# JiLiBIT/LIO-SLAM

Measured on AMD Instinct MI355X. Metric: scan-to-map registrations/sec, 64x1800 scan vs 200-keyframe map; pose RMSE, higher is better.
Workload: dtype f32

## Files before the change

include/liogpu.h:

```cpp
#ifndef LIOGPU_H
#define LIOGPU_H

#include <stddef.h>
#include <stdint.h>

#ifdef __cplusplus
extern "C" {
#endif

#define LIO_VERSION 102
#define LIO_MAX_ITERS 32

enum {
    LIO_OK               = 0,
    LIO_TOO_FEW_POINTS   = 1,
    LIO_TOO_FEW_CORR     = 2,
    LIO_ERR_ARG          = -1,
    LIO_ERR_HIP          = -2,
    LIO_ERR_CAPACITY     = -3,
    LIO_ERR_NO_MAP       = -4,
    LIO_ERR_NO_DEVICE    = -5
};

typedef struct lio_s2m_config {
// ... 56 lines not shown
    float   launch_ms[LIO_MAX_ITERS];
    int32_t launch_active[LIO_MAX_ITERS];
    int64_t point_iters;
    int64_t n_map;
    int64_t n_cells;
    int32_t pipeline;
    int32_t multi_iterations;
    int32_t multi_stream_syncs;
    int32_t multi_event_waits;
    int32_t multi_exchange;
    int32_t persist_fallbacks;
    int32_t map_x_sub;
    int32_t map_tight_tables;
    int32_t map_first_try;
    float   map_pts_per_cell;
} lio_s2m_profile;

typedef struct lio_s2m_handle lio_s2m_handle;

int  lio_version(void);
void lio_s2m_default_config(lio_s2m_config *cfg);
const char *lio_last_error(void);

int  lio_s2m_create(const lio_s2m_config *cfg, lio_s2m_handle **out);
void lio_s2m_destroy(lio_s2m_handle *h);

int  lio_s2m_set_map(lio_s2m_handle *h, const void *pts, size_t n, size_t stride_bytes);

int  lio_s2m_register(lio_s2m_handle *h, const void *scan, size_t n, size_t stride_bytes,
                      float pose[6], lio_s2m_result *res);
// ... 334 lines not shown
```

lio-slam_amd/api.py:

```python
import ctypes as C
import os
import subprocess

import numpy as np

_HERE = os.path.dirname(os.path.abspath(__file__))
LIO_MAX_ITERS = 32
STATUS_NAMES = {0: "OK", 1: "TOO_FEW_POINTS", 2: "TOO_FEW_CORR", -1: "ERR_ARG", -2: "ERR_HIP",
                -3: "ERR_CAPACITY", -4: "ERR_NO_MAP", -5: "ERR_NO_DEVICE"}


class LioError(RuntimeError):
    pass


class S2MConfig(C.Structure):
    _fields_ = [
        ("k", C.c_int32), ("max_sq_dist", C.c_float),
        ("plane_tol", C.c_double), ("weight", C.c_double), ("min_s", C.c_double),
        ("min_corr", C.c_int32), ("max_iters", C.c_int32), ("eig_thresh", C.c_float),
        ("conv_deg", C.c_double), ("conv_cm", C.c_double),
        ("min_scan_pts", C.c_int32), ("jacobian_mode", C.c_int32), ("force_all_iters", C.c_int32),
        ("device_id", C.c_int32), ("cell_size", C.c_float), ("max_batch", C.c_int32),
        ("max_scan_pts", C.c_int32), ("record_corr_iter", C.c_int32), ("kernel_variant", C.c_int32),
# ... 12 lines not shown
        ("matP", C.c_float * 36), ("AtA", C.c_float * 36), ("AtB", C.c_float * 6),
        ("pose_iter", (C.c_float * 6) * LIO_MAX_ITERS),
    ]


class S2MProfile(C.Structure):
    _fields_ = [
        ("map_build_ms", C.c_float), ("map_upload_ms", C.c_float), ("n_launches", C.c_int32),
        ("n_units", C.c_int32), ("unit_iters", C.c_int32),
        ("launch_ms", C.c_float * LIO_MAX_ITERS), ("launch_active", C.c_int32 * LIO_MAX_ITERS),
        ("point_iters", C.c_int64),
        ("n_map", C.c_int64), ("n_cells", C.c_int64),
        ("pipeline", C.c_int32), ("multi_iterations", C.c_int32), ("multi_stream_syncs", C.c_int32),
        ("multi_event_waits", C.c_int32), ("multi_exchange", C.c_int32), ("persist_fallbacks", C.c_int32),
        ("map_x_sub", C.c_int32), ("map_tight_tables", C.c_int32), ("map_first_try", C.c_int32), ("map_pts_per_cell", C.c_float),
    ]


class DeskewConfig(C.Structure):
    _fields_ = [
        ("N_SCAN", C.c_int32), ("downsampleRate", C.c_int32), ("point_filter_num", C.c_int32),
        ("lidarMinFront", C.c_float), ("lidarMinBack", C.c_float),
        ("lidarMinLeft", C.c_float), ("lidarMinRight", C.c_float),
        ("lidarMaxRange", C.c_float), ("lidarMaxIntensity", C.c_float),
        ("deskew_flag", C.c_int32), ("device_id", C.c_int32),
    ]


class RangeImageConfig(C.Structure):
    _fields_ = [("N_SCAN", C.c_int32), ("Horizon_SCAN", C.c_int32), ("downsampleRate", C.c_int32),
# ... 1029 lines not shown
```

lio-slam_amd/csrc/lio_handle.h:

```cpp
#pragma once
#include <hip/hip_runtime.h>
#include <stdio.h>
#include <string.h>
#include <string>
#include <vector>

#include "../../include/liogpu.h"
#include "lio_kernels.h"
#include "lio_pool.h"
#include "lio_types.h"

int lio_pc2_check_xyz(const lio_pc2_layout* L);
void lio_raw_ws_free(struct LioRawWs* ws);

struct lio_s2m_handle {
    ~lio_s2m_handle();
    lio_s2m_config cfg;
    LioConsts c;
    hipStream_t stream = nullptr;
    bool own_stream = true;

    bool has_map = false;
    size_t n_map = 0;
    LioDevBuf<float> d_mx, d_my, d_mz;
// ... 12 lines not shown
    std::vector<LioScanState> h_state;
    std::vector<LioBlockDesc> v_blocks, v_prep;
    std::vector<LioScanTiles> v_tiles;
    std::vector<LioBlockDesc> v_blocks_sorted;
    std::vector<int> v_order, v_first, v_first_orig;
    bool defer_sync = false;
    bool async_upload = false;
    LioDevBuf<float> d_poses;
    const float* reg_pose = nullptr;
    bool pose_in_state = false;
    LioDevBuf<float> d_summary;
    LioPinned<float> h_summary;
    bool host_state_stale = false;
    LioDevBuf<LioBlockDesc> d_blocks;
    int n_blocks = 0, ppt = 1, max_blk = 1;
    LioDevBuf<double> d_partials;
    LioDevBuf<unsigned> d_arrive;
    bool poses_set = false, ran = false;
    LioDevBuf<LioScanTiles> d_tiles;
    LioDevBuf<LioBlockDesc> d_prep_blocks;
    LioDevBuf<int> d_key_of, d_key_count, d_key_start, d_key_tiles, d_tmp_idx, d_perm;
    LioDevBuf<float> d_block_box;
    bool has_block_box = false;
    LioDevBuf<unsigned char> d_blk_skip;
    LioDevBuf<int> d_big_list;
    LioDevBuf<unsigned> d_scan_bbox;
    LioPinned<unsigned> h_scan_bbox;
    bool sorted = false;
    const unsigned char* last_stage = nullptr;
    size_t last_stride = 0, last_xyz_off = 0;
// ... 6 lines not shown
    unsigned persist_spin_max = 0;
    int persist_withhold = -1;
    lio_s2m_handle* map_src = nullptr;
    unsigned long long map_epoch = 0;
    LioDevBuf<float> d_nn_cache;
    LioDevBuf<long long> d_stamps;
    LioDevBuf<unsigned> d_gen;
    LioDevBuf<double> d_spec_sums;
    unsigned gen_epoch = 0;
    int n_cu = 0;
    bool run_persist = false;
    bool soa_valid = true;
    hipGraph_t graph = nullptr;
    hipGraphExec_t graph_exec = nullptr;
    bool graph_dirty = true;
    int graph_chunk = 0, graph_blocks = 0, graph_ppt = 0;
    LioIterParams graph_params;
    int units_this_run = 0, unit_iters = 1;

    LioDevBuf<unsigned char> d_rec_flag;
    LioDevBuf<float> d_rec_coeff;
    LioDevBuf<int> d_rec_nn;

    struct LioMulti* multi = nullptr;

    bool run_pending = false, run_graph = false, run_has_c = false;
    int run_next = 0, run_units = 0, run_look = 0;
    LioIterParams run_P, run_Pc;

    LioShard shard{};
// ... 21 lines not shown
```

lio-slam_amd/csrc/lio_kernels.h:

```cpp
#pragma once
#include <hip/hip_runtime.h>
#include "lio_types.h"

struct LioIterParams {
    LioGrid grid;
    LioShard shard;
    LioConsts c;
    const float4* map_sorted;
    const float4* map_xyz4;
    const int* cell_start;
    const float4* nbr_pts;
    const int* nbr_start;
    const float* sx;
    const float* sy;
    const float* sz;
    const int* perm;
    LioScanState* state;
    const LioBlockDesc* blocks;
    double* partials;
    unsigned* arrive;
    int max_blk;
    int xcd_remap;
    int* n_active;
    double* sums_out;
// ... 6 lines not shown
};

void lio_launch_aos_to_soa(const void* src, size_t stride, int n, float* x, float* y, float* z,
                           float4* xyz4, hipStream_t s);
void lio_launch_map_bbox(const float* x, const float* y, const float* z, int n, unsigned* bbox, hipStream_t s);
void lio_launch_map_build(const LioGrid& g, const float* x, const float* y, const float* z, int n,
                          int* cell_of, int* cell_count, int* cell_start, int* tile_sums,
                          float4* sorted, int* nbr_start, float4* nbr_pts, int* nbr_slot, bool with_cell_sorted, hipStream_t s);
void lio_launch_map_cell_sort(const LioGrid& g, const float* x, const float* y, const float* z, int n, int* cell_of, int* cell_count,
                              int* cell_start, int* tile_sums, float4* sorted, hipStream_t s);
void lio_launch_map_occupancy(const LioGrid& g, const float* x, const float* y, const float* z, int n, int* flags, hipStream_t s);
int  lio_scan_tiles(int n_cells);
void lio_launch_init_state(LioScanState* st, int n_scans, float* poses, bool from_state, const LioConsts& c,
                           int* n_active, hipStream_t s);
void lio_launch_iterate(const LioIterParams& P, int n_blocks, int ppt, bool stage, hipStream_t s, bool corner = false);
void lio_launch_persist(const LioIterParams& P, int n_blocks, unsigned* gen, unsigned epoch, const unsigned char* stage, size_t stride,
                        int n_scans, unsigned* spec, double* spec_sums, const float* poses0, unsigned spin_max, int withhold_wg, hipStream_t s);
void lio_launch_pack_summary(const LioScanState* st, int n_scans, float* out, hipStream_t s);
void lio_launch_apply(LioScanState* st, int n_scans, const double* sums, size_t slot_stride, int n_slots, const LioConsts& c,
                      int* n_active, hipStream_t s);
void lio_launch_shard_cull(const LioIterParams& P, int n_ranks, int rank, int halo, const int* bounds, const float* block_box,
                           int n_blocks, unsigned char* skip, hipStream_t s);
void lio_launch_block_boxes(const LioBlockDesc* blocks, int n_blocks, const LioScanState* st, const float* sx, const float* sy,
                            const float* sz, float* box, hipStream_t s);
void lio_launch_scan_sort_lds(const void* stage, size_t stride, const LioScanState* st, int n_scans, int max_pts, float tile0,
                              int shard_axis, int* perm, float* x, float* y, float* z, hipStream_t s);
void lio_launch_scan_bbox(const void* stage, size_t stride, const LioBlockDesc* prep_blocks, int n_prep_blocks,
                          const LioScanState* st, unsigned* bbox, hipStream_t s);
void lio_launch_scan_tile_sort(const void* stage, size_t stride, int total_pts,
                               const LioBlockDesc* prep_blocks, int n_prep_blocks,
// ... 8 lines not shown
```

lio-slam_amd/csrc/lio_kernels.hip:

```cpp
#include <hip/hip_runtime.h>
#include "lio_types.h"
#include "lio_device_math.h"
#include "lio_kernels.h"

#include "lio_s2m_device.h"
#include "lio_scan2.h"
#include "lio_wg.h"

__global__ void k_aos_to_soa(const unsigned char* __restrict__ src, size_t stride, int n,
                             float* __restrict__ x, float* __restrict__ y, float* __restrict__ z,
                             float4* __restrict__ xyz4 )
{
    int i = blockIdx.x * blockDim.x + threadIdx.x;
    if (i >= n) return;
    const float* p = reinterpret_cast<const float*>(src + (size_t)i * stride);
    const float a = p[0], b = p[1], c = p[2];
    x[i] = a; y[i] = b; z[i] = c;
    if (xyz4) xyz4[i] = make_float4(a, b, c, 0.0f);
}

__global__ void k_xyzi4_to_soa(const float4* __restrict__ src, int n, float* __restrict__ x, float* __restrict__ y,
                               float* __restrict__ z, float4* __restrict__ xyz4)
{
    const int i = blockIdx.x * blockDim.x + threadIdx.x;
// ... 476 lines not shown
    const int li = bd.first + (int)threadIdx.x;
    const int base = st[bd.scan].offset;
    float mn[3] = { INFINITY, INFINITY, INFINITY }, mx[3] = { -INFINITY, -INFINITY, -INFINITY };
    if (li < st[bd.scan].n_pts) {
        const float v[3] = { sx[base + li], sy[base + li], sz[base + li] };
#pragma unroll
        for (int a = 0; a < 3; ++a) if (fabsf(v[a]) <= 3.0e38f) { mn[a] = v[a]; mx[a] = v[a]; }
    }
    __shared__ LioWgBoxLds<LIO_BLOCK / 64> s_box;
    float lo, hi;
    lio_wg_box(mn, mx, s_box, lo, hi);
    if (threadIdx.x < 3) {
        const int a = threadIdx.x;
        float* o = box + (size_t)((base + bd.first) / LIO_BLOCK + bd.scan) * 6;
        o[a] = lo; o[3 + a] = hi;
    }
}

struct LioShardPlan {
    int n_ranks;
    int rank;
    int halo;
    int bounds[9];
};

__global__ __launch_bounds__(256) void k_shard_cull(LioIterParams P, LioShardPlan plan, const float* __restrict__ block_box, int n_blocks,
                                                    unsigned char* __restrict__ skip)
{
    const int lane = threadIdx.x & 63, c = lane & 7;
    const int i = (blockIdx.x * 4 + (int)(threadIdx.x >> 6)) * 8 + (lane >> 3);
// ... 520 lines not shown
    if (stage) {
        switch (ppt) {
        case 1: hipLaunchKernelGGL((k_s2m_iterate<1, true, false>), gr, bl, 0, s, P); break;
        case 2: hipLaunchKernelGGL((k_s2m_iterate<2, true, false>), gr, bl, 0, s, P); break;
        default: hipLaunchKernelGGL((k_s2m_iterate<4, true, false>), gr, bl, 0, s, P); break;
        }
    } else {
        switch (ppt) {
        case 1: hipLaunchKernelGGL((k_s2m_iterate<1, false, false>), gr, bl, 0, s, P); break;
        case 2: hipLaunchKernelGGL((k_s2m_iterate<2, false, false>), gr, bl, 0, s, P); break;
        default: hipLaunchKernelGGL((k_s2m_iterate<4, false, false>), gr, bl, 0, s, P); break;
        }
    }
}

void lio_launch_pack_summary(const LioScanState* st, int n_scans, float* out, hipStream_t s)
{
    hipLaunchKernelGGL(k_s2m_pack_summary, dim3((n_scans + 255) / 256), dim3(256), 0, s, st, n_scans, out);
}

void lio_launch_apply(LioScanState* st, int n_scans, const double* sums, size_t slot_stride, int n_slots, const LioConsts& c,
                      int* n_active, hipStream_t s)
{
    hipLaunchKernelGGL(k_s2m_apply, dim3(n_scans), dim3(64), 0, s, st, n_scans, sums, slot_stride, n_slots, c, n_active);
}

void lio_launch_shard_cull(const LioIterParams& P, int n_ranks, int rank, int halo, const int* bounds, const float* block_box,
                           int n_blocks, unsigned char* skip, hipStream_t s)
{
    if (n_blocks <= 0) return;
// ... 63 lines not shown
```

lio-slam_amd/csrc/liogpu_api.hip:

```cpp
#include <hip/hip_runtime.h>
#include <math.h>
#include <stdio.h>
#include <string.h>
#include <algorithm>
#include <chrono>
#include <exception>
#include <memory>
#include <mutex>
#include <vector>

#include "lio_handle.h"
#include "lio_multi.h"
#include "lio_wg.h"


static thread_local char g_last_error[512];

int lio_fail(int code, const char* what, hipError_t e)
{
    if (e != hipSuccess) snprintf(g_last_error, sizeof(g_last_error), "%s: %s", what, hipGetErrorString(e));
    else snprintf(g_last_error, sizeof(g_last_error), "%s", what);
    return code;
}

// ... 71 lines not shown
}

static int lio_s2m_init_resources(lio_s2m_handle* h)
{
    HIPCHK(hipStreamCreateWithFlags(&h->stream, hipStreamNonBlocking));
    for (int i = 0; i < LIO_MAX_ITERS; ++i) {
        HIPCHK(hipEventCreate(&h->ev_beg[i]));
        HIPCHK(hipEventCreate(&h->ev_end[i]));
        HIPCHK(hipEventCreateWithFlags(&h->ev_chk[i], hipEventDisableTiming));
    }
    HIPCHK(h->h_active.grow(LIO_MAX_ITERS, LIO_MAX_ITERS));
    HIPCHK(hipEventCreate(&h->ev_map[0]));
    HIPCHK(hipEventCreate(&h->ev_map[1]));
    HIPCHK(hipEventCreate(&h->ev_mapl[0]));
    HIPCHK(hipEventCreate(&h->ev_mapl[1]));
    HIPCHK(h->d_bbox.grow(6, 1.0, 0));
    HIPCHK(h->d_active.grow(1, 1.0, 0));
    hipDeviceProp_t prop;
    if (hipGetDeviceProperties(&prop, h->cfg.device_id) == hipSuccess) h->n_cu = prop.multiProcessorCount;
    (void)hipGetLastError();
    return LIO_OK;
}

extern "C" int lio_s2m_create(const lio_s2m_config* cfg, lio_s2m_handle** out)
try {
    if (!cfg || !out) return lio_fail(LIO_ERR_ARG, "null argument");
    if (cfg->k != 5) return lio_fail(LIO_ERR_ARG, "only k = 5 is supported (MO:1631)");
    if (cfg->max_iters < 1 || cfg->max_iters > LIO_MAX_ITERS) return lio_fail(LIO_ERR_ARG, "max_iters out of range");
    if (!(cfg->max_sq_dist > 0.0f)) return lio_fail(LIO_ERR_ARG, "max_sq_dist must be positive");
    if (cfg->x_sub != 0 && cfg->x_sub != 1 && cfg->x_sub != 2 && cfg->x_sub != 4 && cfg->x_sub != 8)
// ... 30 lines not shown
    (void)hipSetDevice(h->cfg.device_id);
    (void)hipStreamSynchronize(h->stream);
    delete h;
}

lio_s2m_handle::~lio_s2m_handle()
{
    delete multi;
    lio_s2m_destroy(corner);
    lio_raw_ws_free(raw_ws);
    for (int i = 0; i < LIO_MAX_ITERS; ++i) {
        if (ev_beg[i]) (void)hipEventDestroy(ev_beg[i]);
        if (ev_end[i]) (void)hipEventDestroy(ev_end[i]);
        if (ev_chk[i]) (void)hipEventDestroy(ev_chk[i]);
    }
    for (hipEvent_t e : { ev_map[0], ev_map[1], ev_mapl[0], ev_mapl[1] }) if (e) (void)hipEventDestroy(e);
    if (graph_exec) (void)hipGraphExecDestroy(graph_exec);
    if (graph) (void)hipGraphDestroy(graph);
    if (own_stream && stream) (void)hipStreamDestroy(stream);
}

extern "C" int lio_s2m_set_stream(lio_s2m_handle* h, void* hip_stream)
try {
    if (h && h->multi) return lio_fail(LIO_ERR_ARG, "not available on a multi-device handle (cfg.n_devices > 1 shards inside the library)");
    if (!h) return lio_fail(LIO_ERR_ARG, "null handle");
    HIPCHK(hipStreamSynchronize(h->stream));
    if (h->own_stream && h->stream) HIPCHK(hipStreamDestroy(h->stream));
    h->stream = (hipStream_t)hip_stream;
    h->own_stream = false;
    h->graph_dirty = true;
    if (h->corner) return lio_s2m_set_stream(h->corner, hip_stream);
// ... 142 lines not shown
        h->prof.map_build_ms = ms;
        h->map_timing_pending = false;
        HIPCHK(hipEventRecord(h->ev_mapl[1], h->stream));
    }
    h->prof.map_upload_ms = std::chrono::duration<float, std::milli>(t1 - t0).count();
    h->prof.n_map = (int64_t)n;
    h->prof.n_cells = g.n_cells;
    h->prof.map_x_sub = g.xs;
    h->prof.map_tight_tables = n_tb;
    h->prof.map_first_try = g.tb_try;
    h->prof.map_pts_per_cell = pts_per_cell;
    h->n_map = n;
    h->has_map = true;
    h->graph_dirty = true;
    h->map_epoch++;
    return LIO_OK;
}

extern "C" int lio_s2m_set_map(lio_s2m_handle* h, const void* pts, size_t n, size_t stride)
try {
    if (!h) return lio_fail(LIO_ERR_ARG, "null handle");
    if (n > 0 && !pts) return lio_fail(LIO_ERR_ARG, "null map pointer");
    if (stride < 12 || (stride & 3)) return lio_fail(LIO_ERR_ARG, "stride_bytes must be >= 12 and a multiple of 4");
    if (h->multi) return lio_multi_set_map(h, pts, n, stride);
    if (n >= (1ull << 25)) return lio_fail(LIO_ERR_CAPACITY, "map too large ((2k+1)^2 x n records must fit a 31-bit offset)");
    if (h->map_src) return lio_fail(LIO_ERR_ARG, "this handle searches another handle's map (lio_s2m_share_map)");
    HIPCHK(hipSetDevice(h->cfg.device_id));
    (void)hipGetLastError();
    auto t0 = std::chrono::steady_clock::now();
    h->has_map = false;
// ... 197 lines not shown
    lio_launch_debug_plane_fit(d_sets, (long long)n, plane_tol, d_out, nullptr);
    HIPCHK(hipGetLastError());
    HIPCHK(hipMemcpy(out, d_out, n * 8 * sizeof(unsigned), hipMemcpyDeviceToHost));
    return LIO_OK;
} LIO_CATCH

static int lio_ensure_soa(lio_s2m_handle* h)
{
    if (h->soa_valid || !h->total_pts) return LIO_OK;
    lio_launch_aos_to_soa(h->last_stage + h->last_xyz_off, h->last_stride, (int)h->total_pts, h->d_sx, h->d_sy, h->d_sz, nullptr, h->stream);
    h->soa_valid = true;
    HIPCHK(hipGetLastError());
    return LIO_OK;
}

extern "C" int lio_s2m_batch_upload(lio_s2m_handle* h, int32_t n_scans, const void* const* scans,
                                    const size_t* n_pts, size_t stride)
try {
    if (!h || !scans || !n_pts) return lio_fail(LIO_ERR_ARG, "null argument");
    if (n_scans < 1) return lio_fail(LIO_ERR_ARG, "n_scans must be >= 1");
    if (stride < 12 || (stride & 3)) return lio_fail(LIO_ERR_ARG, "stride_bytes must be >= 12 and a multiple of 4");
    if (h->multi) return lio_multi_upload(h, n_scans, scans, n_pts, stride);
    HIPCHK(hipSetDevice(h->cfg.device_id));
    (void)hipGetLastError();
    size_t total = 0, max_n = 0;
    for (int s = 0; s < n_scans; ++s) {
        if (n_pts[s] && !scans[s]) return lio_fail(LIO_ERR_ARG, "null scan pointer");
        total += n_pts[s];
        if (n_pts[s] > max_n) max_n = n_pts[s];
    }
    if (total > 0x7fffffffull - 1024) return lio_fail(LIO_ERR_CAPACITY, "batch too large");
    h->run_pending = false;
    if (h->host_state_stale && h->n_scans > 0 && h->d_state) {
        HIPCHK(hipMemcpyAsync(h->h_state.data(), h->d_state, (size_t)h->n_scans * sizeof(LioScanState),
                              hipMemcpyDeviceToHost, h->stream));
        HIPCHK(hipStreamSynchronize(h->stream));
    }
    h->host_state_stale = false;
    const size_t tt = total ? total : 1;
    HIPCHK(h->d_sx.grow(tt));
    HIPCHK(h->d_sy.grow(tt));
    HIPCHK(h->d_sz.grow(tt));
    HIPCHK(h->d_stage.grow(tt * stride));
    HIPCHK(h->d_state.grow((size_t)n_scans));
    HIPCHK(h->d_poses.grow((size_t)n_scans * 6));
    {
        bool fresh = false;
        HIPCHK(h->d_arrive.grow((size_t)n_scans, 1.25, 64, false, &fresh));
        if (fresh) HIPCHK(hipMemsetAsync(h->d_arrive, 0, h->d_arrive.cap * sizeof(unsigned), h->stream));
    }
    if (h->cfg.nn_cache && !h->cfg.use_lds) HIPCHK(h->d_nn_cache.grow(tt));

    int ppt = h->cfg.kernel_variant;
    if (ppt != 1 && ppt != 2 && ppt != 4) ppt = 1;
    h->ppt = ppt;
    const size_t per_blk = (size_t)LIO_BLOCK * ppt;
    std::vector<LioBlockDesc>& blocks = h->v_blocks;
    blocks.clear();
    int max_blk = 1;
    const size_t old_scans = h->h_state.size();
    h->h_state.resize((size_t)n_scans);
    size_t off = 0;
    for (int s = 0; s < n_scans; ++s) {
        LioScanState& st = h->h_state[s];
        if ((size_t)s >= old_scans) memset(&st, 0, sizeof(st));
        st.n_pts = (int)n_pts[s];
        st.offset = (int)off;
        if (h->reg_pose && n_scans == 1) memcpy(st.pose, h->reg_pose, sizeof(float) * 6);
        st.c_n_pts = 0;
        st.c_offset = 0;
        st.done = 1;
        const int nb = (int)((n_pts[s] + per_blk - 1) / per_blk);
        const int bw = h->block_world > 1 ? h->block_world : 1, br = h->block_world > 1 ? h->block_rank : 0;
        const int part = (br + s) % bw;
        const int b0 = (int)((long long)nb * part / bw), b1 = (int)((long long)nb * (part + 1) / bw);
        const int nb_local = b1 - b0;
        if (nb_local > max_blk) max_blk = nb_local;
        for (int b = b0; b < b1; ++b) blocks.push_back({ s, (int)(b * per_blk), b - b0, nb_local });
        off += n_pts[s];
    }
    const unsigned char* stage = h->d_stage;
    bool host_copy = false;
    {
        bool contiguous = true;
        for (int s = 0; s + 1 < n_scans && contiguous; ++s)
            contiguous = (const unsigned char*)scans[s + 1] == (const unsigned char*)scans[s] + n_pts[s] * stride;
        bool in_place = false;
        if (contiguous && total) {
            hipPointerAttribute_t at;
            if (hipPointerGetAttributes(&at, scans[0]) == hipSuccess)
                in_place = at.type == hipMemoryTypeDevice && at.device == h->cfg.device_id;
            (void)hipGetLastError();
        }
        if (in_place) {
            stage = (const unsigned char*)scans[0];
        } else if (contiguous && total) {
            HIPCHK(hipMemcpyAsync(h->d_stage, scans[0], total * stride, hipMemcpyDefault, h->stream));
            host_copy = true;
        } else {
            host_copy = true;
            size_t o = 0;
            for (int s = 0; s < n_scans; ++s) {
                if (n_pts[s])
                    HIPCHK(hipMemcpyAsync(h->d_stage + o * stride, scans[s], n_pts[s] * stride, hipMemcpyDefault, h->stream));
                o += n_pts[s];
            }
        }
    }
    if (host_copy && h->async_upload) {
        HIPCHK(hipEventRecord(h->ev_map[0], h->stream));
        HIPCHK(hipEventSynchronize(h->ev_map[0]));
    }
    h->last_stage = stage; h->last_stride = stride; h->last_xyz_off = h->xyz_off;
    h->last_int_off = h->int_off != -2 ? h->int_off : ((h->xyz_off == 0 && stride >= 20) ? 16 : -1);
    h->int_off = -2;
    stage += h->xyz_off;
    h->xyz_off = 0;
    h->v_first_orig.assign((size_t)n_scans + 1, 0);
    for (const LioBlockDesc& b : blocks) h->v_first_orig[b.scan + 1]++;
    for (int s = 0; s < n_scans; ++s) h->v_first_orig[s + 1] += h->v_first_orig[s];
    h->n_scans = n_scans;
    h->total_pts = total;
    h->n_blocks = (int)blocks.size();
    h->max_blk = max_blk;
    HIPCHK(h->d_blocks.grow(blocks.size() ? blocks.size() : 1));
    HIPCHK(h->d_partials.grow((size_t)n_scans * max_blk * LIO_SUMS));
    if (h->cfg.profile == 2) {
        HIPCHK(h->d_stamps.grow(blocks.size() * (LIO_BLOCK / 64) * 8 + 8));
        HIPCHK(hipMemsetAsync(h->d_stamps, 0, (blocks.size() * (LIO_BLOCK / 64) * 8 + 8) * sizeof(long long), h->stream));
    }
    if (h->cfg.record_corr_iter >= 0) {
        HIPCHK(h->d_rec_flag.grow(tt));
        HIPCHK(h->d_rec_coeff.grow(tt * 4));
        HIPCHK(h->d_rec_nn.grow(tt * 5));
        HIPCHK(hipMemsetAsync(h->d_rec_flag, 0, tt, h->stream));
        HIPCHK(hipMemsetAsync(h->d_rec_coeff, 0, tt * 4 * sizeof(float), h->stream));
        HIPCHK(hipMemsetAsync(h->d_rec_nn, 0xff, tt * 5 * sizeof(int), h->stream));
    }
    if (!blocks.empty())
        HIPCHK(hipMemcpyAsync(h->d_blocks, blocks.data(), blocks.size() * sizeof(LioBlockDesc),
                              hipMemcpyHostToDevice, h->stream));
    HIPCHK(hipMemcpyAsync(h->d_state, h->h_state.data(), (size_t)n_scans * sizeof(LioScanState),
                          hipMemcpyHostToDevice, h->stream));
    std::vector<LioScanTiles>& tiles = h->v_tiles;
    std::vector<LioBlockDesc>& prep = h->v_prep;
    tiles.clear(); prep.clear();
    h->sorted = false;
    const bool want_sort = total && (h->cfg.sort_scan >= 2 || (h->cfg.sort_scan == 1 && total >= 65536));
    if (want_sort && max_n < 16384 && h->cfg.sort_scan != 3) {
        HIPCHK(h->d_perm.grow(tt));
        lio_launch_scan_sort_lds(stage, stride, h->d_state, n_scans, (int)max_n, h->cfg.tile_size > 0.0f ? h->cfg.tile_size : 4.0f,
                                 h->shard.axis, h->d_perm, h->d_sx, h->d_sy, h->d_sz, h->stream);
        h->sorted = true;
    } else if (want_sort) {
        for (int s = 0; s < n_scans; ++s) {
            const int nb1 = (int)((n_pts[s] + LIO_BLOCK - 1) / LIO_BLOCK);
            for (int b = 0; b < nb1; ++b) prep.push_back({ s, b * LIO_BLOCK, b, nb1 });
        }
// ... 97 lines not shown

extern "C" int lio_s2m_batch_upload_corners(lio_s2m_handle* h, int32_t n_scans, const void* const* scans,
                                            const size_t* n_pts, size_t stride)
try {
    if (!h || !scans || !n_pts) return lio_fail(LIO_ERR_ARG, "null argument");
    if (!h->corner || !h->corner->has_map) return lio_fail(LIO_ERR_NO_MAP, "set_corner_map has not been called");
    if (h->n_scans < 1 || n_scans != h->n_scans)
        return lio_fail(LIO_ERR_ARG, "upload the surf batch first; the corner batch must have the same number of scans");
    lio_s2m_handle* ch = h->corner;
    ch->block_rank = h->block_rank;
    ch->block_world = h->block_world;
    ch->defer_sync = h->defer_sync;
    int rc = lio_s2m_batch_upload(ch, n_scans, scans, n_pts, stride);
    ch->defer_sync = false;
    if (rc != LIO_OK) return rc;
    int max_blk = 1;
    for (LioBlockDesc& b : h->v_blocks) {
        const int ns = h->v_first_orig[b.scan + 1] - h->v_first_orig[b.scan];
        const int nc = ch->v_first_orig[b.scan + 1] - ch->v_first_orig[b.scan];
        b.n_blk = ns + nc;
        if (b.n_blk > max_blk) max_blk = b.n_blk;
    }
    for (LioBlockDesc& b : ch->v_blocks) {
        const int ns = h->v_first_orig[b.scan + 1] - h->v_first_orig[b.scan];
        const int nc = ch->v_first_orig[b.scan + 1] - ch->v_first_orig[b.scan];
        b.blk += ns;
        b.n_blk = ns + nc;
        if (b.n_blk > max_blk) max_blk = b.n_blk;
    }
    h->max_blk = max_blk;
// ... 22 lines not shown
try {
    if (!h) return lio_fail(LIO_ERR_ARG, "null handle");
    if (!h->corner || !h->corner_active) return lio_fail(LIO_ERR_ARG, "no corner batch is resident");
    return lio_s2m_get_correspondences(h->corner, scan, flag, coeff4, nn_idx5);
} LIO_CATCH

extern "C" int lio_s2m_batch_set_poses(lio_s2m_handle* h, const float* poses)
try {
    if (!h || !poses) return lio_fail(LIO_ERR_ARG, "null argument");
    if (h->n_scans < 1) return lio_fail(LIO_ERR_ARG, "no batch uploaded");
    if (h->multi) return lio_multi_set_poses(h, poses);
    HIPCHK(hipSetDevice(h->cfg.device_id));
    (void)hipGetLastError();
    h->run_pending = false;
    h->pose_in_state = false;
    HIPCHK(hipMemcpyAsync(h->d_poses, poses, (size_t)h->n_scans * 6 * sizeof(float), hipMemcpyHostToDevice, h->stream));
    if (h->cfg.sort_batch && h->n_scans > 8 && !h->v_blocks.empty()) {
        const LioGrid& mg = lio_map_of(h)->grid;
        const float ext[3] = { (float)mg.nx, (float)mg.ny, (float)mg.nz };
        const int ax = (ext[0] >= ext[1] && ext[0] >= ext[2]) ? 0 : (ext[1] >= ext[2] ? 1 : 2);
        std::vector<int>& order = h->v_order;
        order.resize((size_t)h->n_scans);
        for (int s = 0; s < h->n_scans; ++s) order[s] = s;
        std::stable_sort(order.begin(), order.end(),
                         [&](int a, int b) { return poses[a * 6 + 3 + ax] < poses[b * 6 + 3 + ax]; });
        std::vector<int>& first = h->v_first;
        first.assign((size_t)h->n_scans + 1, 0);
        for (const LioBlockDesc& b : h->v_blocks) first[b.scan + 1]++;
        for (int s = 0; s < h->n_scans; ++s) first[s + 1] += first[s];
        std::vector<LioBlockDesc>& sorted = h->v_blocks_sorted;
        sorted.clear();
        sorted.reserve(h->v_blocks.size());
        for (int k = 0; k < h->n_scans; ++k) {
            const int s = order[k];
            for (int i = h->v_first_orig[s]; i < h->v_first_orig[s + 1]; ++i) sorted.push_back(h->v_blocks[i]);
        }
        HIPCHK(hipMemcpyAsync(h->d_blocks, sorted.data(), sorted.size() * sizeof(LioBlockDesc), hipMemcpyHostToDevice, h->stream));
    }
    if (!h->defer_sync) HIPCHK(hipStreamSynchronize(h->stream));
    h->poses_set = true;
    return LIO_OK;
} LIO_CATCH

extern "C" int lio_s2m_set_degeneracy(lio_s2m_handle* h, int32_t scan, const float matP[36], int32_t is_degenerate)
try {
    if (!h || !matP) return lio_fail(LIO_ERR_ARG, "null argument");
    if (scan < 0 || scan >= h->n_scans) return lio_fail(LIO_ERR_ARG, "scan slot out of range");
    if (h->multi) return lio_multi_set_degeneracy(h, scan, matP, is_degenerate);
    HIPCHK(hipSetDevice(h->cfg.device_id));
    (void)hipGetLastError();
    LioScanState& st = h->h_state[scan];
    memcpy(st.matP, matP, sizeof(float) * 36);
    st.is_degenerate = is_degenerate;
    char* base = (char*)(h->d_state + scan);
// ... 51 lines not shown
    if (Pc) lio_launch_iterate(*Pc, h->corner->n_blocks, 1, false, h->stream, true);
    lio_launch_iterate(P, h->n_blocks, h->ppt, h->cfg.use_lds != 0, h->stream);
}

extern "C" int lio_s2m_batch_begin(lio_s2m_handle* h)
try {
    if (h && h->multi) return lio_fail(LIO_ERR_ARG, "not available on a multi-device handle (cfg.n_devices > 1 shards inside the library)");
    if (!h) return lio_fail(LIO_ERR_ARG, "null handle");
    if (!lio_map_of(h)->has_map) return lio_fail(LIO_ERR_NO_MAP, "set_map has not been called");
    if (h->n_scans < 1 || !h->poses_set) return lio_fail(LIO_ERR_ARG, "batch_upload and batch_set_poses first");
    HIPCHK(hipSetDevice(h->cfg.device_id));
    (void)hipGetLastError();
    if (h->map_src && h->map_epoch != h->map_src->map_epoch) {
        h->map_epoch = h->map_src->map_epoch;
        h->graph_dirty = true;
        HIPCHK(hipStreamWaitEvent(h->stream, h->map_src->ev_mapl[1], 0));
    }
    lio_launch_init_state(h->d_state, h->n_scans, h->d_poses, h->pose_in_state, h->c, h->d_active, h->stream);
    h->pose_in_state = false;
    if (h->cfg.nn_cache && !h->cfg.use_lds && h->d_nn_cache && h->shard.axis >= 0)
        HIPCHK(hipMemsetAsync(h->d_nn_cache, 0xff, (h->total_pts ? h->total_pts : 1) * sizeof(float), h->stream));
    if (h->corner_active && h->corner->d_nn_cache && h->shard.axis >= 0)
        HIPCHK(hipMemsetAsync(h->corner->d_nn_cache, 0xff, (h->corner->total_pts ? h->corner->total_pts : 1) * sizeof(float), h->stream));
    h->launches_this_run = 0;
    h->units_this_run = 0;
    h->unit_iters = 1;
    h->ran = true;
    return LIO_OK;
} LIO_CATCH

static int lio_graph_prepare(lio_s2m_handle* h, const LioIterParams& P, const LioIterParams* Pc, int chunk)
{
    const int nbc = Pc ? h->corner->n_blocks : -1;
    if (h->graph_exec && h->graph_chunk == chunk && h->graph_blocks == h->n_blocks && h->graph_ppt == h->ppt &&
        memcmp(&h->graph_params, &P, sizeof(P)) == 0 && h->graph_blocks_c == nbc &&
        (!Pc || memcmp(&h->graph_params_c, Pc, sizeof(P)) == 0))
        return LIO_OK;
    if (h->graph_exec) { HIPCHK(hipGraphExecDestroy(h->graph_exec)); h->graph_exec = nullptr; }
    if (h->graph) { HIPCHK(hipGraphDestroy(h->graph)); h->graph = nullptr; }
    HIPCHK(hipStreamBeginCapture(h->stream, hipStreamCaptureModeThreadLocal));
    for (int i = 0; i < chunk; ++i) lio_launch_gn(h, P, Pc);
    HIPCHK(hipStreamEndCapture(h->stream, &h->graph));
    HIPCHK(hipGraphInstantiate(&h->graph_exec, h->graph, nullptr, nullptr, 0));
    h->graph_chunk = chunk; h->graph_blocks = h->n_blocks; h->graph_ppt = h->ppt;
    memcpy(&h->graph_params, &P, sizeof(P));
    h->graph_blocks_c = nbc;
    if (Pc) memcpy(&h->graph_params_c, Pc, sizeof(P));
    h->graph_dirty = false;
    return LIO_OK;
}

static int lio_run_continue(lio_s2m_handle* h, bool blocking)
{
    if (!h->run_pending) return LIO_OK;
    const bool prof = h->cfg.profile != 0;
    const LioIterParams* Pc = h->run_has_c ? &h->run_Pc : nullptr;
    while (h->run_next < h->run_units && h->run_next < LIO_MAX_ITERS) {
        const int u = h->run_next;
        const int chk = u - 1 - h->run_look;
        if (chk >= 0) {
            if (blocking) {
                HIPCHK(hipEventSynchronize(h->ev_chk[chk]));
            } else {
                const hipError_t q = hipEventQuery(h->ev_chk[chk]);
                if (q == hipErrorNotReady) { (void)hipGetLastError(); return LIO_OK; }
                HIPCHK(q);
            }
            if (h->h_active[chk] == 0) break;
        }
        if (prof) HIPCHK(hipEventRecord(h->ev_beg[u], h->stream));
        if (h->run_persist) {
            lio_launch_persist(h->run_P, h->n_blocks, h->d_gen, h->gen_epoch, h->soa_valid ? nullptr : h->last_stage + h->last_xyz_off,
                               h->last_stride, h->n_scans, getenv("LIO_NO_SPEC") ? nullptr : h->d_gen + h->n_scans, h->d_spec_sums, h->d_poses,
                               lio_persist_spin_max(h), h->persist_withhold, h->stream);
        } else if (h->run_graph) HIPCHK(hipGraphLaunch(h->graph_exec, h->stream));
        else lio_launch_gn(h, h->run_P, Pc);
        if (prof) HIPCHK(hipEventRecord(h->ev_end[u], h->stream));
        if (!h->run_persist) HIPCHK(hipMemcpyAsync(&h->h_active[u], h->d_active, sizeof(int), hipMemcpyDeviceToHost, h->stream));
        HIPCHK(hipEventRecord(h->ev_chk[u], h->stream));
        h->run_next = u + 1;
        h->units_this_run = u + 1;
        h->launches_this_run = (u + 1) * h->unit_iters;
    }
    h->run_pending = false;
    HIPCHK(hipGetLastError());
    return LIO_OK;
}

extern "C" int lio_s2m_batch_run(lio_s2m_handle* h)
try {
// ... 541 lines not shown
```

Before: 438,100.

## Move batch state and block-list setup to device, update graphs in place

Per-scan state staging and the sorted block list are now built on the device by small kernels, fed from pinned host buffers. This replaces host-side block vectors and full state copies, and removes the stream synchronize in set_poses. The iterate graph is built from explicit kernel nodes and refreshed with hipGraphExecKernelNodeSetParams instead of being recaptured and reinstantiated. Pointer-attribute lookups are cached per base pointer. The aim is to cut host-side latency per batch, at the cost of more complex state-validity bookkeeping (lazy host blocks, stale host state) and a single-workgroup block-list kernel.

```diff
diff --git a/include/liogpu.h b/include/liogpu.h
--- a/include/liogpu.h
+++ b/include/liogpu.h
@@ -94,6 +94,10 @@
     int32_t map_tight_tables;
     int32_t map_first_try;
     float   map_pts_per_cell;
+    int32_t graph_builds;
+    int32_t graph_updates;
+    float   graph_build_ms;
+    float   graph_update_ms;
 } lio_s2m_profile;
 
 typedef struct lio_s2m_handle lio_s2m_handle;
diff --git a/lio-slam_amd/api.py b/lio-slam_amd/api.py
--- a/lio-slam_amd/api.py
+++ b/lio-slam_amd/api.py
@@ -50,6 +50,7 @@
         ("pipeline", C.c_int32), ("multi_iterations", C.c_int32), ("multi_stream_syncs", C.c_int32),
         ("multi_event_waits", C.c_int32), ("multi_exchange", C.c_int32), ("persist_fallbacks", C.c_int32),
         ("map_x_sub", C.c_int32), ("map_tight_tables", C.c_int32), ("map_first_try", C.c_int32), ("map_pts_per_cell", C.c_float),
+        ("graph_builds", C.c_int32), ("graph_updates", C.c_int32), ("graph_build_ms", C.c_float), ("graph_update_ms", C.c_float),
     ]
 
 
diff --git a/lio-slam_amd/csrc/lio_handle.h b/lio-slam_amd/csrc/lio_handle.h
--- a/lio-slam_amd/csrc/lio_handle.h
+++ b/lio-slam_amd/csrc/lio_handle.h
@@ -50,6 +50,16 @@
     bool host_state_stale = false;
     LioDevBuf<LioBlockDesc> d_blocks;
     int n_blocks = 0, ppt = 1, max_blk = 1;
+    LioPinned<int> h_np_off;
+    LioDevBuf<int> d_np_off;
+    LioPinned<float> h_pose_stage;
+    hipEvent_t ev_np = nullptr, ev_pose = nullptr;
+    bool ev_np_armed = false, ev_pose_armed = false;
+    bool state_on_device = false;
+    bool list_deferred = false;
+    bool host_blocks_valid = false;
+    const void* attr_base = nullptr;
+    bool attr_in_place = false;
     LioDevBuf<double> d_partials;
     LioDevBuf<unsigned> d_arrive;
     bool poses_set = false, ran = false;
@@ -86,6 +96,10 @@
     hipGraph_t graph = nullptr;
     hipGraphExec_t graph_exec = nullptr;
     bool graph_dirty = true;
+    std::vector<hipGraphNode_t> graph_nodes;
+    bool graph_stage = false;
+    int graph_last_unit = -1;
+    bool graph_update_refused = false;
     int graph_chunk = 0, graph_blocks = 0, graph_ppt = 0;
     LioIterParams graph_params;
     int units_this_run = 0, unit_iters = 1;
diff --git a/lio-slam_amd/csrc/lio_kernels.h b/lio-slam_amd/csrc/lio_kernels.h
--- a/lio-slam_amd/csrc/lio_kernels.h
+++ b/lio-slam_amd/csrc/lio_kernels.h
@@ -44,6 +44,10 @@
 void lio_launch_init_state(LioScanState* st, int n_scans, float* poses, bool from_state, const LioConsts& c,
                            int* n_active, hipStream_t s);
 void lio_launch_iterate(const LioIterParams& P, int n_blocks, int ppt, bool stage, hipStream_t s, bool corner = false);
+const void* lio_iterate_kernel(int ppt, bool stage, bool corner);
+void lio_launch_stage_state(LioScanState* st, int n_scans, const int* np_off, hipStream_t s);
+void lio_launch_block_list(const LioScanState* st, const int* order, int n_scans, int per_blk, LioBlockDesc* blocks, int cap,
+                           hipStream_t s);
 void lio_launch_persist(const LioIterParams& P, int n_blocks, unsigned* gen, unsigned epoch, const unsigned char* stage, size_t stride,
                         int n_scans, unsigned* spec, double* spec_sums, const float* poses0, unsigned spin_max, int withhold_wg, hipStream_t s);
 void lio_launch_pack_summary(const LioScanState* st, int n_scans, float* out, hipStream_t s);
diff --git a/lio-slam_amd/csrc/lio_kernels.hip b/lio-slam_amd/csrc/lio_kernels.hip
--- a/lio-slam_amd/csrc/lio_kernels.hip
+++ b/lio-slam_amd/csrc/lio_kernels.hip
@@ -514,6 +514,38 @@
         const int a = threadIdx.x;
         float* o = box + (size_t)((base + bd.first) / LIO_BLOCK + bd.scan) * 6;
         o[a] = lo; o[3 + a] = hi;
+    }
+}
+
+__global__ void k_s2m_stage_state(LioScanState* __restrict__ st, int n_scans, const int* __restrict__ np_off)
+{
+    const int s = blockIdx.x * blockDim.x + threadIdx.x;
+    if (s >= n_scans) return;
+    LioScanState* p = &st[s];
+    p->n_pts = np_off[s];
+    p->offset = np_off[n_scans + s];
+    p->c_n_pts = 0;
+    p->c_offset = 0;
+    p->done = 1;
+}
+
+__global__ __launch_bounds__(256) void k_s2m_block_list(const LioScanState* __restrict__ st, const int* __restrict__ order, int n_scans,
+                                                        int per_blk, LioBlockDesc* __restrict__ blocks, int cap)
+{
+    __shared__ int s_wave[4];
+    int carry = 0;
+    for (int b = 0; b < n_scans; b += 256) {
+        const int k = b + (int)threadIdx.x;
+        const int s = k < n_scans ? order[k] : 0;
+        const int nb = k < n_scans ? (st[s].n_pts + per_blk - 1) / per_blk : 0;
+        int tot;
+        const int at = carry + lio_wg_exclusive_scan<4>(nb, &tot, s_wave);
+        carry += tot;
+        for (int i = 0; i < nb && at + i < cap; ++i) {
+            LioBlockDesc d;
+            d.scan = s; d.first = i * per_blk; d.blk = i; d.n_blk = nb;
+            blocks[at + i] = d;
+        }
     }
 }
 
@@ -1064,6 +1096,36 @@
     }
 }
 
+const void* lio_iterate_kernel(int ppt, bool stage, bool corner)
+{
+    if (corner) return (const void*)&k_s2m_iterate<1, false, true>;
+    if (stage) {
+        switch (ppt) {
+        case 1: return (const void*)&k_s2m_iterate<1, true, false>;
+        case 2: return (const void*)&k_s2m_iterate<2, true, false>;
+        default: return (const void*)&k_s2m_iterate<4, true, false>;
+        }
+    }
+    switch (ppt) {
+    case 1: return (const void*)&k_s2m_iterate<1, false, false>;
+    case 2: return (const void*)&k_s2m_iterate<2, false, false>;
+    default: return (const void*)&k_s2m_iterate<4, false, false>;
+    }
+}
+
+void lio_launch_stage_state(LioScanState* st, int n_scans, const int* np_off, hipStream_t s)
+{
+    if (n_scans <= 0) return;
+    hipLaunchKernelGGL(k_s2m_stage_state, dim3((n_scans + 255) / 256), dim3(256), 0, s, st, n_scans, np_off);
+}
+
+void lio_launch_block_list(const LioScanState* st, const int* order, int n_scans, int per_blk, LioBlockDesc* blocks, int cap,
+                           hipStream_t s)
+{
+    if (n_scans <= 0 || cap <= 0) return;
+    hipLaunchKernelGGL(k_s2m_block_list, dim3(1), dim3(256), 0, s, st, order, n_scans, per_blk, blocks, cap);
+}
+
 void lio_launch_pack_summary(const LioScanState* st, int n_scans, float* out, hipStream_t s)
 {
     hipLaunchKernelGGL(k_s2m_pack_summary, dim3((n_scans + 255) / 256), dim3(256), 0, s, st, n_scans, out);
diff --git a/lio-slam_amd/csrc/liogpu_api.hip b/lio-slam_amd/csrc/liogpu_api.hip
--- a/lio-slam_amd/csrc/liogpu_api.hip
+++ b/lio-slam_amd/csrc/liogpu_api.hip
@@ -109,6 +109,8 @@
     HIPCHK(hipEventCreate(&h->ev_map[1]));
     HIPCHK(hipEventCreate(&h->ev_mapl[0]));
     HIPCHK(hipEventCreate(&h->ev_mapl[1]));
+    HIPCHK(hipEventCreateWithFlags(&h->ev_np, hipEventDisableTiming));
+    HIPCHK(hipEventCreateWithFlags(&h->ev_pose, hipEventDisableTiming));
     HIPCHK(h->d_bbox.grow(6, 1.0, 0));
     HIPCHK(h->d_active.grow(1, 1.0, 0));
     hipDeviceProp_t prop;
@@ -169,7 +171,7 @@
         if (ev_end[i]) (void)hipEventDestroy(ev_end[i]);
         if (ev_chk[i]) (void)hipEventDestroy(ev_chk[i]);
     }
-    for (hipEvent_t e : { ev_map[0], ev_map[1], ev_mapl[0], ev_mapl[1] }) if (e) (void)hipEventDestroy(e);
+    for (hipEvent_t e : { ev_map[0], ev_map[1], ev_mapl[0], ev_mapl[1], ev_np, ev_pose }) if (e) (void)hipEventDestroy(e);
     if (graph_exec) (void)hipGraphExecDestroy(graph_exec);
     if (graph) (void)hipGraphDestroy(graph);
     if (own_stream && stream) (void)hipStreamDestroy(stream);
@@ -342,6 +344,7 @@
     h->has_map = true;
     h->graph_dirty = true;
     h->map_epoch++;
+    h->attr_base = nullptr;
     return LIO_OK;
 }
 
@@ -569,6 +572,31 @@
     return LIO_OK;
 }
 
+static int lio_refresh_host_state(lio_s2m_handle* h)
+{
+    if (h->host_state_stale && h->n_scans > 0 && h->d_state) {
+        HIPCHK(hipMemcpyAsync(h->h_state.data(), h->d_state, (size_t)h->n_scans * sizeof(LioScanState),
+                              hipMemcpyDeviceToHost, h->stream));
+        HIPCHK(hipStreamSynchronize(h->stream));
+    }
+    h->host_state_stale = false;
+    return LIO_OK;
+}
+
+static void lio_host_blocks(lio_s2m_handle* h)
+{
+    if (h->host_blocks_valid) return;
+    const int per_blk = LIO_BLOCK * h->ppt;
+    h->v_blocks.clear();
+    h->v_first_orig.assign((size_t)h->n_scans + 1, 0);
+    for (int s = 0; s < h->n_scans; ++s) {
+        const int nb = (h->h_state[s].n_pts + per_blk - 1) / per_blk;
+        for (int b = 0; b < nb; ++b) h->v_blocks.push_back({ s, b * per_blk, b, nb });
+        h->v_first_orig[s + 1] = h->v_first_orig[s] + nb;
+    }
+    h->host_blocks_valid = true;
+}
+
 extern "C" int lio_s2m_batch_upload(lio_s2m_handle* h, int32_t n_scans, const void* const* scans,
                                     const size_t* n_pts, size_t stride)
 try {
@@ -586,19 +614,25 @@
     }
     if (total > 0x7fffffffull - 1024) return lio_fail(LIO_ERR_CAPACITY, "batch too large");
     h->run_pending = false;
-    if (h->host_state_stale && h->n_scans > 0 && h->d_state) {
-        HIPCHK(hipMemcpyAsync(h->h_state.data(), h->d_state, (size_t)h->n_scans * sizeof(LioScanState),
-                              hipMemcpyDeviceToHost, h->stream));
-        HIPCHK(hipStreamSynchronize(h->stream));
-    }
-    h->host_state_stale = false;
+    const bool state_on_device = !(h->reg_pose && n_scans == 1);
+    if (!state_on_device) { const int rcs = lio_refresh_host_state(h); if (rcs != LIO_OK) return rcs; }
     const size_t tt = total ? total : 1;
     HIPCHK(h->d_sx.grow(tt));
     HIPCHK(h->d_sy.grow(tt));
     HIPCHK(h->d_sz.grow(tt));
     HIPCHK(h->d_stage.grow(tt * stride));
-    HIPCHK(h->d_state.grow((size_t)n_scans));
-    HIPCHK(h->d_poses.grow((size_t)n_scans * 6));
+    if (!h->d_state || (size_t)n_scans > h->d_state.cap) {
+        LioDevBuf<LioScanState> grown;
+        HIPCHK(grown.grow((size_t)n_scans));
+        HIPCHK(hipMemsetAsync(grown, 0, grown.cap * sizeof(LioScanState), h->stream));
+        if (h->d_state && h->n_scans > 0)
+            HIPCHK(hipMemcpyAsync(grown, h->d_state, (size_t)h->n_scans * sizeof(LioScanState), hipMemcpyDeviceToDevice, h->stream));
+        HIPCHK(hipStreamSynchronize(h->stream));
+        h->d_state = std::move(grown);
+    } else if (n_scans > h->n_scans) {
+        HIPCHK(hipMemsetAsync(h->d_state + h->n_scans, 0, (size_t)(n_scans - h->n_scans) * sizeof(LioScanState), h->stream));
+    }
+    HIPCHK(h->d_poses.grow((size_t)n_scans * 7));
     {
         bool fresh = false;
         HIPCHK(h->d_arrive.grow((size_t)n_scans, 1.25, 64, false, &fresh));
@@ -610,22 +644,37 @@
     if (ppt != 1 && ppt != 2 && ppt != 4) ppt = 1;
     h->ppt = ppt;
     const size_t per_blk = (size_t)LIO_BLOCK * ppt;
+    const bool list_deferred = h->cfg.sort_batch && n_scans > 8 && h->block_world <= 1 && h->shard.axis < 0;
     std::vector<LioBlockDesc>& blocks = h->v_blocks;
     blocks.clear();
-    int max_blk = 1;
+    int max_blk = 1, n_blocks = 0;
     const size_t old_scans = h->h_state.size();
     h->h_state.resize((size_t)n_scans);
+    int* np_off = nullptr;
+    if (state_on_device) {
+        if (h->ev_np_armed) { HIPCHK(hipEventSynchronize(h->ev_np)); h->ev_np_armed = false; }
+        HIPCHK(h->h_np_off.grow((size_t)n_scans * 2, (size_t)n_scans * 2 + 128));
+        HIPCHK(h->d_np_off.grow((size_t)n_scans * 2));
+        np_off = h->h_np_off;
+    }
     size_t off = 0;
     for (int s = 0; s < n_scans; ++s) {
         LioScanState& st = h->h_state[s];
         if ((size_t)s >= old_scans) memset(&st, 0, sizeof(st));
         st.n_pts = (int)n_pts[s];
         st.offset = (int)off;
+        if (np_off) { np_off[s] = st.n_pts; np_off[n_scans + s] = st.offset; }
         if (h->reg_pose && n_scans == 1) memcpy(st.pose, h->reg_pose, sizeof(float) * 6);
         st.c_n_pts = 0;
         st.c_offset = 0;
         st.done = 1;
         const int nb = (int)((n_pts[s] + per_blk - 1) / per_blk);
+        if (list_deferred) {
+            if (nb > max_blk) max_blk = nb;
+            n_blocks += nb;
+            off += n_pts[s];
+            continue;
+        }
         const int bw = h->block_world > 1 ? h->block_world : 1, br = h->block_world > 1 ? h->block_rank : 0;
         const int part = (br + s) % bw;
         const int b0 = (int)((long long)nb * part / bw), b1 = (int)((long long)nb * (part + 1) / bw);
@@ -642,10 +691,15 @@
             contiguous = (const unsigned char*)scans[s + 1] == (const unsigned char*)scans[s] + n_pts[s] * stride;
         bool in_place = false;
         if (contiguous && total) {
-            hipPointerAttribute_t at;
-            if (hipPointerGetAttributes(&at, scans[0]) == hipSuccess)
-                in_place = at.type == hipMemoryTypeDevice && at.device == h->cfg.device_id;
-            (void)hipGetLastError();
+            if (scans[0] == h->attr_base && h->attr_in_place) {
+                in_place = true;
+            } else {
+                hipPointerAttribute_t at;
+                if (hipPointerGetAttributes(&at, scans[0]) == hipSuccess)
+                    in_place = at.type == hipMemoryTypeDevice && at.device == h->cfg.device_id;
+                (void)hipGetLastError();
+                h->attr_base = scans[0]; h->attr_in_place = in_place;
+            }
         }
         if (in_place) {
             stage = (const unsigned char*)scans[0];
@@ -671,18 +725,24 @@
     h->int_off = -2;
     stage += h->xyz_off;
     h->xyz_off = 0;
-    h->v_first_orig.assign((size_t)n_scans + 1, 0);
-    for (const LioBlockDesc& b : blocks) h->v_first_orig[b.scan + 1]++;
-    for (int s = 0; s < n_scans; ++s) h->v_first_orig[s + 1] += h->v_first_orig[s];
+    if (!list_deferred) {
+        n_blocks = (int)blocks.size();
+        h->v_first_orig.assign((size_t)n_scans + 1, 0);
+        for (const LioBlockDesc& b : blocks) h->v_first_orig[b.scan + 1]++;
+        for (int s = 0; s < n_scans; ++s) h->v_first_orig[s + 1] += h->v_first_orig[s];
+    }
+    h->host_blocks_valid = !list_deferred;
+    h->list_deferred = list_deferred;
+    h->state_on_device = state_on_device;
     h->n_scans = n_scans;
     h->total_pts = total;
-    h->n_blocks = (int)blocks.size();
+    h->n_blocks = n_blocks;
     h->max_blk = max_blk;
-    HIPCHK(h->d_blocks.grow(blocks.size() ? blocks.size() : 1));
+    HIPCHK(h->d_blocks.grow(n_blocks ? (size_t)n_blocks : 1));
     HIPCHK(h->d_partials.grow((size_t)n_scans * max_blk * LIO_SUMS));
     if (h->cfg.profile == 2) {
-        HIPCHK(h->d_stamps.grow(blocks.size() * (LIO_BLOCK / 64) * 8 + 8));
-        HIPCHK(hipMemsetAsync(h->d_stamps, 0, (blocks.size() * (LIO_BLOCK / 64) * 8 + 8) * sizeof(long long), h->stream));
+        HIPCHK(h->d_stamps.grow((size_t)n_blocks * (LIO_BLOCK / 64) * 8 + 8));
+        HIPCHK(hipMemsetAsync(h->d_stamps, 0, ((size_t)n_blocks * (LIO_BLOCK / 64) * 8 + 8) * sizeof(long long), h->stream));
     }
     if (h->cfg.record_corr_iter >= 0) {
         HIPCHK(h->d_rec_flag.grow(tt));
@@ -695,8 +755,16 @@
     if (!blocks.empty())
         HIPCHK(hipMemcpyAsync(h->d_blocks, blocks.data(), blocks.size() * sizeof(LioBlockDesc),
                               hipMemcpyHostToDevice, h->stream));
-    HIPCHK(hipMemcpyAsync(h->d_state, h->h_state.data(), (size_t)n_scans * sizeof(LioScanState),
-                          hipMemcpyHostToDevice, h->stream));
+    if (state_on_device) {
+        HIPCHK(hipMemcpyAsync(h->d_np_off, np_off, (size_t)n_scans * 2 * sizeof(int), hipMemcpyHostToDevice, h->stream));
+        HIPCHK(hipEventRecord(h->ev_np, h->stream));
+        h->ev_np_armed = true;
+        lio_launch_stage_state(h->d_state, n_scans, h->d_np_off, h->stream);
+    } else {
+        HIPCHK(hipMemcpyAsync(h->d_state, h->h_state.data(), (size_t)n_scans * sizeof(LioScanState),
+                              hipMemcpyHostToDevice, h->stream));
+        h->host_state_stale = false;
+    }
     std::vector<LioScanTiles>& tiles = h->v_tiles;
     std::vector<LioBlockDesc>& prep = h->v_prep;
     tiles.clear(); prep.clear();
@@ -824,6 +892,11 @@
     int rc = lio_s2m_batch_upload(ch, n_scans, scans, n_pts, stride);
     ch->defer_sync = false;
     if (rc != LIO_OK) return rc;
+    lio_host_blocks(h);
+    lio_host_blocks(ch);
+    if ((rc = lio_refresh_host_state(h)) != LIO_OK) return rc;
+    h->list_deferred = false;
+    ch->list_deferred = false;
     int max_blk = 1;
     for (LioBlockDesc& b : h->v_blocks) {
         const int ns = h->v_first_orig[b.scan + 1] - h->v_first_orig[b.scan];
@@ -876,8 +949,31 @@
     (void)hipGetLastError();
     h->run_pending = false;
     h->pose_in_state = false;
-    HIPCHK(hipMemcpyAsync(h->d_poses, poses, (size_t)h->n_scans * 6 * sizeof(float), hipMemcpyHostToDevice, h->stream));
-    if (h->cfg.sort_batch && h->n_scans > 8 && !h->v_blocks.empty()) {
+    const size_t n6 = (size_t)h->n_scans * 6;
+    if (h->ev_pose_armed) { HIPCHK(hipEventSynchronize(h->ev_pose)); h->ev_pose_armed = false; }
+    HIPCHK(h->h_pose_stage.grow((size_t)h->n_scans * 7, (size_t)h->n_scans * 7 + 448));
+    memcpy(h->h_pose_stage, poses, n6 * sizeof(float));
+    const bool reorder = h->cfg.sort_batch && h->n_scans > 8 && h->n_blocks > 0;
+    const bool on_device = reorder && h->list_deferred;
+    if (on_device) {
+        const LioGrid& mg = lio_map_of(h)->grid;
+        const float ext[3] = { (float)mg.nx, (float)mg.ny, (float)mg.nz };
+        const int ax = (ext[0] >= ext[1] && ext[0] >= ext[2]) ? 0 : (ext[1] >= ext[2] ? 1 : 2);
+        std::vector<int>& order = h->v_order;
+        order.resize((size_t)h->n_scans);
+        for (int s = 0; s < h->n_scans; ++s) order[s] = s;
+        std::stable_sort(order.begin(), order.end(),
+                         [&](int a, int b) { return poses[a * 6 + 3 + ax] < poses[b * 6 + 3 + ax]; });
+        memcpy(h->h_pose_stage + n6, order.data(), (size_t)h->n_scans * sizeof(int));
+    }
+    HIPCHK(hipMemcpyAsync(h->d_poses, h->h_pose_stage, (on_device ? (size_t)h->n_scans * 7 : n6) * sizeof(float), hipMemcpyHostToDevice, h->stream));
+    HIPCHK(hipEventRecord(h->ev_pose, h->stream));
+    h->ev_pose_armed = true;
+    if (on_device) {
+        lio_launch_block_list(h->d_state, (const int*)(h->d_poses + n6), h->n_scans, LIO_BLOCK * h->ppt, h->d_blocks, h->n_blocks, h->stream);
+        HIPCHK(hipGetLastError());
+    } else if (reorder) {
+        lio_host_blocks(h);
         const LioGrid& mg = lio_map_of(h)->grid;
         const float ext[3] = { (float)mg.nx, (float)mg.ny, (float)mg.nz };
         const int ax = (ext[0] >= ext[1] && ext[0] >= ext[2]) ? 0 : (ext[1] >= ext[2] ? 1 : 2);
@@ -898,8 +994,8 @@
             for (int i = h->v_first_orig[s]; i < h->v_first_orig[s + 1]; ++i) sorted.push_back(h->v_blocks[i]);
         }
         HIPCHK(hipMemcpyAsync(h->d_blocks, sorted.data(), sorted.size() * sizeof(LioBlockDesc), hipMemcpyHostToDevice, h->stream));
-    }
-    if (!h->defer_sync) HIPCHK(hipStreamSynchronize(h->stream));
+        if (!h->defer_sync) HIPCHK(hipStreamSynchronize(h->stream));
+    }
     h->poses_set = true;
     return LIO_OK;
 } LIO_CATCH
@@ -981,6 +1077,7 @@
     if (h->map_src && h->map_epoch != h->map_src->map_epoch) {
         h->map_epoch = h->map_src->map_epoch;
         h->graph_dirty = true;
+        h->attr_base = nullptr;
         HIPCHK(hipStreamWaitEvent(h->stream, h->map_src->ev_mapl[1], 0));
     }
     lio_launch_init_state(h->d_state, h->n_scans, h->d_poses, h->pose_in_state, h->c, h->d_active, h->stream);
@@ -999,21 +1096,66 @@
 static int lio_graph_prepare(lio_s2m_handle* h, const LioIterParams& P, const LioIterParams* Pc, int chunk)
 {
     const int nbc = Pc ? h->corner->n_blocks : -1;
-    if (h->graph_exec && h->graph_chunk == chunk && h->graph_blocks == h->n_blocks && h->graph_ppt == h->ppt &&
-        memcmp(&h->graph_params, &P, sizeof(P)) == 0 && h->graph_blocks_c == nbc &&
+    const bool stage = h->cfg.use_lds != 0;
+    const bool same_shape = h->graph_exec && h->graph_chunk == chunk && h->graph_ppt == h->ppt && h->graph_stage == stage &&
+                            (h->graph_blocks_c >= 0) == (nbc >= 0);
+    if (same_shape && h->graph_blocks == h->n_blocks && memcmp(&h->graph_params, &P, sizeof(P)) == 0 && h->graph_blocks_c == nbc &&
         (!Pc || memcmp(&h->graph_params_c, Pc, sizeof(P)) == 0))
         return LIO_OK;
-    if (h->graph_exec) { HIPCHK(hipGraphExecDestroy(h->graph_exec)); h->graph_exec = nullptr; }
-    if (h->graph) { HIPCHK(hipGraphDestroy(h->graph)); h->graph = nullptr; }
-    HIPCHK(hipStreamBeginCapture(h->stream, hipStreamCaptureModeThreadLocal));
-    for (int i = 0; i < chunk; ++i) lio_launch_gn(h, P, Pc);
-    HIPCHK(hipStreamEndCapture(h->stream, &h->graph));
-    HIPCHK(hipGraphInstantiate(&h->graph_exec, h->graph, nullptr, nullptr, 0));
-    h->graph_chunk = chunk; h->graph_blocks = h->n_blocks; h->graph_ppt = h->ppt;
+    const bool timed = h->cfg.profile != 0;
+    const auto t0 = timed ? std::chrono::steady_clock::now() : std::chrono::steady_clock::time_point();
+    LioIterParams args = P, args_c = Pc ? *Pc : P;
+    void* kp[1] = { &args }; void* kpc[1] = { &args_c };
+    hipKernelNodeParams np = {}, npc = {};
+    np.func = const_cast<void*>(lio_iterate_kernel(h->ppt, stage, false));
+    np.gridDim = dim3((unsigned)h->n_blocks); np.blockDim = dim3(LIO_BLOCK); np.sharedMemBytes = 0; np.kernelParams = kp; np.extra = nullptr;
+    npc = np;
+    npc.func = const_cast<void*>(lio_iterate_kernel(1, false, true));
+    npc.gridDim = dim3((unsigned)(nbc > 0 ? nbc : 1)); npc.kernelParams = kpc;
+    bool updated = false;
+    if (same_shape && !h->graph_update_refused) {
+        if (h->graph_last_unit >= 0) HIPCHK(hipEventSynchronize(h->ev_chk[h->graph_last_unit]));
+        hipError_t e = hipSuccess;
+        size_t i = 0;
+        for (int it = 0; it < chunk && e == hipSuccess; ++it) {
+            if (Pc) e = hipGraphExecKernelNodeSetParams(h->graph_exec, h->graph_nodes[i++], &npc);
+            if (e == hipSuccess) e = hipGraphExecKernelNodeSetParams(h->graph_exec, h->graph_nodes[i++], &np);
+        }
+        updated = e == hipSuccess;
+        if (updated) {
+            h->prof.graph_updates++;
+        } else {
+            (void)hipGetLastError();
+            h->graph_update_refused = true;
+            fprintf(stderr, "[liogpu] the runtime refused to update the executable graph in place (%s): this handle instantiates a new "
+                            "graph per batch from now on\n", hipGetErrorString(e));
+        }
+    }
+    if (!updated) {
+        if (h->graph_exec) { HIPCHK(hipGraphExecDestroy(h->graph_exec)); h->graph_exec = nullptr; }
+        if (h->graph) { HIPCHK(hipGraphDestroy(h->graph)); h->graph = nullptr; }
+        h->graph_nodes.clear();
+        HIPCHK(hipGraphCreate(&h->graph, 0));
+        for (int it = 0; it < chunk; ++it) {
+            for (int c = Pc ? 0 : 1; c < 2; ++c) {
+                hipGraphNode_t node = nullptr;
+                const hipGraphNode_t* dep = h->graph_nodes.empty() ? nullptr : &h->graph_nodes.back();
+                HIPCHK(hipGraphAddKernelNode(&node, h->graph, dep, dep ? 1 : 0, c == 0 ? &npc : &np));
+                h->graph_nodes.push_back(node);
+            }
+        }
+        HIPCHK(hipGraphInstantiate(&h->graph_exec, h->graph, nullptr, nullptr, 0));
+        h->prof.graph_builds++;
+    }
+    h->graph_chunk = chunk; h->graph_blocks = h->n_blocks; h->graph_ppt = h->ppt; h->graph_stage = stage;
     memcpy(&h->graph_params, &P, sizeof(P));
     h->graph_blocks_c = nbc;
     if (Pc) memcpy(&h->graph_params_c, Pc, sizeof(P));
     h->graph_dirty = false;
+    if (timed) {
+        const float ms = std::chrono::duration<float, std::milli>(std::chrono::steady_clock::now() - t0).count();
+        if (updated) h->prof.graph_update_ms += ms; else h->prof.graph_build_ms += ms;
+    }
     return LIO_OK;
 }
 
@@ -1040,7 +1182,7 @@
             lio_launch_persist(h->run_P, h->n_blocks, h->d_gen, h->gen_epoch, h->soa_valid ? nullptr : h->last_stage + h->last_xyz_off,
                                h->last_stride, h->n_scans, getenv("LIO_NO_SPEC") ? nullptr : h->d_gen + h->n_scans, h->d_spec_sums, h->d_poses,
                                lio_persist_spin_max(h), h->persist_withhold, h->stream);
-        } else if (h->run_graph) HIPCHK(hipGraphLaunch(h->graph_exec, h->stream));
+        } else if (h->run_graph) { HIPCHK(hipGraphLaunch(h->graph_exec, h->stream)); h->graph_last_unit = u; }
         else lio_launch_gn(h, h->run_P, Pc);
         if (prof) HIPCHK(hipEventRecord(h->ev_end[u], h->stream));
         if (!h->run_persist) HIPCHK(hipMemcpyAsync(&h->h_active[u], h->d_active, sizeof(int), hipMemcpyDeviceToHost, h->stream));
```

Result: no change. 442,200, median of 6 (+1.0%).
